# enyen/dppo

Hardware: AMD Instinct MI355X
Metric: PPO-update samples/sec (+ env-steps/sec of the K=20 sampler), hopper K=20 n_envs=512 (higher is better)
Workload: dtype bf16; 1 GPU; hopper-medium-v2 ft_ppo_diffusion_mlp K=20 Kft=10 Ta=4 (BASELINE configs[1]); n_envs_per_gpu=512, minibatch_per_gpu=50000, rollout_rows_per_gpu=256000, parallelism=dp1 (env-sharded, RCCL grad all-reduce)

## Files before the change

dppo_amd/csrc/api.hip:

```cpp
#include <math.h>
#include <stdarg.h>
#include <stdio.h>
#include <string.h>

#include "fused.h"
#include "gemm.h"
#include "ppo.h"
#include "gaussian.h"
#include "gmm.h"
#include "unet.h"
#include "sampler.h"

using namespace dppo;

static thread_local char g_err[512] = "";
static int fail(int code, const char* fmt, ...) {
  va_list ap;
  va_start(ap, fmt);
  vsnprintf(g_err, sizeof(g_err), fmt, ap);
  va_end(ap);
  return code;
}
namespace dppo {
void set_vis_mfma_attn(int v);
// ... 577 lines not shown
  return g_lowrank_top && d.n_blocks >= 1 && M >= (int64_t)g_lowrank_ratio * d.out_dim;
}
static int g_mom_rider = 0;
constexpr int64_t MOM_RIDER_MAX_N = 16384;
static int g_temb_onehot = 1;
template <class P>
static int temb_onehot_col(const dppo_net_desc& d, const PackLayout& L, int Kft, const MlpBufs<P>& B) {
  if (!g_temb_onehot || d.kind != 0 || !fused_ok<P>(d) || Kft < 1) return -1;
  if (d.cond_out > 0 && d.cond_out % 16) return -1;
  if (L.Kp0 - d.in_dim < Kft || (size_t)(d.hidden + d.time_dim) * Kft > B.part_floats) return -1;
  return d.in_dim;
}
static int g_dw0 = 1;
static int g_side_tail = 1;
static int g_tail_post = 1;
static int dw0_cols(const dppo_net_desc& d) { return d.kind == 0 ? d.act_flat + d.cond_dim : d.in_dim; }
static int dw0_nhot(const dppo_net_desc& d, int Kft) {
  const int room = 32 - dw0_cols(d);
  return d.kind != 0 ? 0 : (room >= Kft ? Kft : room);
}
template <class P>
static bool dw0_ok(const dppo_net_desc& d, int64_t M, const PackLayout& L, int Kft, const MlpBufs<P>& B, bool wants_dobs) {
  if (!g_dw0 || P::ESIZE != 2 || wants_dobs || d.cond_hidden > 0 || !g_tn_group || !g_post_one) return false;
  if (!fused_ok<P>(d) || B.tiles <= 0 || !bwd_one<P>(d, M) || !fused_dw0_shape(d) || L.Kp0 < 64) return false;
  if (d.kind == 0) {
    if (temb_onehot_col<P>(d, L, Kft, B) < 0 || !B.post_zeroed || d.in_dim != d.act_flat + d.time_dim + d.cond_dim) return false;
    if (d.act_flat % 4 || d.time_dim % 4 || 32 + d.time_dim > 64) return false;
    if (dw0_nhot(d, Kft) < Kft - 1) return false;
  } else if (d.in_dim > 32) {
    return false;
  }
  return (size_t)fused_bwd_one_grid<P>(d, M) * d.hidden * 32 <= B.slab_floats / 2;
}
template <class P>
static void flush_slabs(MlpBufs<P>& B, hipStream_t s, const SlotOuts* slots = nullptr, int slot_width = 0,
                        const LossArgs* fin = nullptr, bool defer_reduce = false) {
  if (B.tn_group.n > 0) {
    GemmTNGroup& gr = B.tn_group;
    gemm_tn_group_order(gr);
    launch_gemm_tn_group<P>(gr, s);
    gr.n = 0;
  }
  for (int i = 0; i + 1 < B.n_join; ++i) join_side(B.join_s[B.n_join - 1], B.join_s[i], B.join_idx[i]);
  if (B.n_join > 0) join_side(s, B.join_s[B.n_join - 1], B.join_idx[B.n_join - 1]);
  B.n_join = 0;
  if (defer_reduce) return;
  if (slots != nullptr || fin != nullptr) {
    TailReduce t;
    memset(&t, 0, sizeof(t));
    t.jobs = B.slab_jobs;
    if (slots != nullptr) t.colsum = B.tile_colsum, t.tiles = B.tiles, t.width = slot_width, t.slots = *slots;
    if (g_dbg & 4) t.jobs.n = 0;
    if (g_dbg & 8) t.slots.n_slots = 0;
    if (g_dbg & 16) fin = nullptr;
    launch_tail_reduce(t, fin, s);
  } else {
    launch_slab_reduce_batch(B.slab_jobs, s);
  }
  B.slab_jobs.n = 0, B.slab_used = 0;
}
template <class P>
static void weight_grad(const void* A, int lda, int N1, const void* Bm, int ldb, int N2, int64_t M, MlpBufs<P>& B,
                        float* gw, int ldgw, hipStream_t s, bool defer = false, int n2a = -1, float* gw2 = nullptr,
                        int ldgw2 = 0) {
  const bool swap = N1 <= 64 && N2 > 64;
  if (swap) {
// ... 81 lines not shown
  g.X = B.d_enc, g.W = pk + L.Wc2T, g.out_pre = B.d_cz, g.dsrc_kind = 2, g.dsrc_ld = L.C1p, g.dact = d.act;
  g.dsrc = d.act == DPPO_ACT_RELU ? B.ca : B.cz;
  launch_gemm_nt<P>(g, s);
  weight_grad<P>(B.d_cz, L.C1p, d.cond_hidden, cin, L.Kpc, d.cond_dim, M, B, grad + pl.c1w, d.cond_dim, s);
  launch_colsum<P>(B.d_cz, (int)M, d.cond_hidden, L.C1p, B.part, REDUCE_BLOCKS, grad + pl.c1b, 1.f, s);
}

template <class P>
static void mlp_backward(const dppo_net_desc& d, const float* prm, const char* pk, const PackLayout& L, int64_t M,
                         MlpBufs<P>& B, float* grad, const int32_t* krow, const dppo_step* ksteps, int Kft,
                         hipStream_t s, bool bout_done = false, int aux_idx = 1, const LossArgs* fin = nullptr) {
  const ParamLayout pl = param_layout(d);
  const int H = d.hidden, nb = d.n_blocks;
  if (fused_ok<P>(d) && B.tiles > 0) {
    FusedBwdArgs f;
    memset(&f, 0, sizeof(f));
    const FusedGeom fg = fused_geom<P>(d);
    f.bstream = (const u32x4*)(pk + L.bstream), f.d_out = B.d_out, f.ld_dout = L.Kpo, f.M = (int)M, f.KpB0 = fg.KpB0;
    f.nb = nb, f.act = d.act, f.colsum = B.tile_colsum, f.out_valid = d.out_dim;
    f.dout_slot = bout_done ? -1 : 2 * nb + 1 + (d.use_layernorm ? 4 * nb : 0);
    const bool post = false;
    f.params = prm, f.use_ln = d.use_layernorm, f.ln_stats = B.ln_stats;
    if (d.use_layernorm) fill_ln_off(d, pl, f.ln_off);
    for (int b = 0; b < nb; ++b) {
      f.m1[b] = post ? B.a2[b] : B.z1[b];
      f.m0[b] = post ? B.a1[b] : B.hpre[b];
      f.dz1[b] = B.dz1_all[b];
    }
    for (int b = 0; b <= nb; ++b) f.dh[b] = B.dh_all[b];
    const bool lowrank = lowrank_top(d, M);
    if (lowrank) f.dh[nb] = nullptr;
    const bool one = bwd_one<P>(d, M);
    f.one_block = one ? 1 : 0;
    if (g_dbg & 1)
      for (int b = 0; b <= nb; ++b) f.dh[b] = nullptr, f.dz1[b < nb ? b : 0] = nullptr;
    if (g_dbg & 32) f.dh[0] = nullptr;
    if (g_dbg & 2)
      for (int b = 0; b < nb; ++b) f.m1[b] = f.m0[b] = nullptr;
    const bool dw0 = B.dw0 && one && !(g_dbg & 33);
    const int dw0_nh = dw0 ? dw0_nhot(d, Kft) : 0;
    float* dw0_slab = nullptr;
    int dw0_grid = 0;
    if (B.dw0 && !dw0) {
      g_fused_fault = -7;
      return;
    }
    if (dw0) {
      dw0_grid = fused_bwd_one_grid<P>(d, M);
      if ((size_t)dw0_grid * H * 32 > B.slab_floats - B.slab_used) flush_slabs(B, s);
      dw0_slab = B.slab + B.slab_used;
      B.slab_used += (size_t)dw0_grid * H * 32;
      f.dh[0] = nullptr, f.dw0_slab = dw0_slab, f.xc = B.in, f.ld_xc = L.Kp0;
      f.xc_af = d.kind == 0 ? d.act_flat : 64, f.xc_skip = d.kind == 0 ? d.time_dim : 0;
      f.dw0_round = d.kind == 0 && dw0_nh < Kft ? 1 : 0;
    }
    g_fused_fault = launch_fused_backward<P>(d, f, s);
    if (g_fused_fault != 0) return;
    {
      SlotOuts so;
      memset(&so, 0, sizeof(so));
      so.n_slots = 2 * nb + 1;
      for (int b = nb - 1; b >= 0; --b) {
        so.out[nb - (b + 1)] = grad + pl.l2b[b];
        so.out[(nb + 1) + (nb - 1 - b)] = grad + pl.l1b[b];
      }
      so.out[nb] = grad + pl.b0;
      if (d.use_layernorm) {
        for (int b = nb - 1; b >= 0; --b) {
          const int ls = (2 * nb + 1) + 4 * (nb - 1 - b);
          so.out[ls] = grad + pl.n1w[b], so.out[ls + 1] = grad + pl.n1b[b];
          so.out[ls + 2] = grad + pl.n2w[b], so.out[ls + 3] = grad + pl.n2b[b];
        }
        so.n_slots += 4 * nb;
      }
      for (int i = 0; i < so.n_slots; ++i) so.n[i] = H;
      if (one) so.n[0] = 0;
      const float* s_rest = dw0 && f.dw0_round ? grad + pl.b0 : nullptr;
      if (!bout_done) so.out[so.n_slots] = grad + pl.bout, so.n[so.n_slots] = d.out_dim, ++so.n_slots;
      const int oh = d.kind == 0 ? temb_onehot_col<P>(d, L, Kft, B) : -1;
      const bool need_aux = d.kind == 0 && oh < 0;
      hipStream_t aux = aux_idx >= 0 && need_aux ? fork_side(s, aux_idx) : s;
      if (need_aux) time_embedding_grad<P>(d, prm, pk, L, M, B, B.dh_all[0], grad, krow, ksteps, Kft, aux);
      const bool merged = B.merged;
      const bool side_tail = dw0 && d.kind == 0 && oh >= 0 && aux_idx >= 0 && !need_aux && g_side_tail && g_early_join && g_post_one &&
                             B.post_zeroed && !(g_dbg & 28);
      TailReduce side_t;
      memset(&side_t, 0, sizeof(side_t));
      if (merged)
        weight_grad<P>(B.d_out, L.Kpo, d.out_dim, B.in, L.Kp0, d.in_dim, M, B, B.lowrank_u, L.Kp0, s, true);
      else
        weight_grad<P>(B.d_out, L.Kpo, d.out_dim, B.hE, H, H, M, B, grad + pl.Wout, H, s, true);
      for (int b = nb - 1; b >= 0; --b) {
        if ((lowrank || merged) && b == nb - 1)
          weight_grad<P>(B.d_out, L.Kpo, d.out_dim, B.a2[b], H, H, M, B, B.lowrank, H, s, true);
        if (!(lowrank && b == nb - 1))
          weight_grad<P>(B.dh_all[b + 1], H, H, B.a2[b], H, H, M, B, grad + pl.l2w[b], H, s, true);
        weight_grad<P>(B.dz1_all[b], H, H, B.a1[b], H, H, M, B, grad + pl.l1w[b], H, s, true);
      }
      if (dw0) {
        auto job = [&](int c0, int cols, float* out, int ldo) {
          SlabJob& j = side_tail ? side_t.jobs.j[side_t.jobs.n++] : B.slab_jobs.j[B.slab_jobs.n++];
          j.slab = dw0_slab, j.out = out, j.splits = dw0_grid, j.rows = H, j.cols = cols, j.lds = 32, j.ldo = ldo, j.transpose = 0;
          j.c0 = c0, j.wide = dw0_grid >= 32 ? 1 : 0;
        };
        if (d.kind == 0) {
          job(0, d.act_flat, grad + pl.W0, d.in_dim);
          job(d.act_flat, d.cond_dim, grad + pl.W0 + d.act_flat + d.time_dim, d.in_dim);
          job(d.act_flat + d.cond_dim, dw0_nh, B.part, Kft);
        } else {
          job(0, d.in_dim, grad + pl.W0, d.in_dim);
        }
      } else if (g_dbg & 32) {
      } else if (oh >= 0)
        weight_grad<P>(B.dh_all[0], H, H, B.in, L.Kp0, d.in_dim + Kft, M, B, grad + pl.W0, d.in_dim, s, true, d.in_dim, B.part,
                       Kft);
      else
        weight_grad<P>(B.dh_all[0], H, H, B.in, L.Kp0, d.in_dim, M, B, grad + pl.W0, d.in_dim, s, true);
      if (side_tail) {
        hipStream_t st = fork_side(s, aux_idx);
        side_t.colsum = B.tile_colsum, side_t.tiles = B.tiles, side_t.width = H, side_t.slots = so;
        launch_tail_reduce(side_t, fin, st);
        PostReduce qs;
        memset(&qs, 0, sizeof(qs));
        qs.H = H, qs.out_dim = d.out_dim;
        qs.S = B.part, qs.W0 = prm + pl.W0, qs.ldw0 = d.in_dim, qs.AF = d.act_flat, qs.Kft = Kft, qs.td = d.time_dim;
        qs.G = B.part + (size_t)H * Kft, qs.w1 = prm + pl.te1_w, qs.b1 = prm + pl.te1_b, qs.w2 = prm + pl.te2_w;
        qs.ksteps = ksteps, qs.gw1 = grad + pl.te1_w, qs.gb1 = grad + pl.te1_b, qs.gw2 = grad + pl.te2_w, qs.gb2 = grad + pl.te2_b;
        qs.S_rest = s_rest, qs.dW0t = grad + pl.W0, qs.temb = (const float*)(pk + L.temb), qs.temb_bf16 = P::ESIZE == 2 ? 1 : 0;
        qs.counter = (unsigned*)B.post_counter;
        launch_post_reduce(qs, st);
// ... 1601 lines not shown
      g_tn_max_splits = value;
      return 0;
    case 5: set_gemm_tn_variant(value); return 0;
    case 6: set_gemm_tn_thin(value); return 0;
    case 7: set_fused_short_tiles(value); return 0;
    case 8: g_dbg = value; return 0;
    case 9: case 10: return retired_knob(knob);
    case 11: g_temb_onehot = value; return 0;
    case 12: g_tn_group = value; return 0;
    case 13: g_pack_one = value; return 0;
    case 14: g_early_join = value; return 0;
    case 15: set_sampler_l0_lds(value); return 0;
    case 16: g_lowrank_top = value; return 0;
    case 17: g_merge_top = value; return 0;
    case 18: g_post_one = value; return 0;
    case 20: dppo::set_vis_mfma_attn(value); return 0;
    case 21: set_gemm_nt_small(value); return 0;
    case 22: set_fused_merge_fwd(value); return 0;
    case 23: set_fused_bwd_one(value); return 0;
    case 25: set_fused_compact(value); return 0;
    case 26: set_gemm_tn_nbuf(value); return 0;
    case 27: set_sampler_split(value); return 0;
    case 28: set_sampler_split_pre_sweep(value); return 0;
    case 29: set_sampler_split_spin_limit(value); return 0;
    case 30:
      if (value < 1) break;
      g_lowrank_ratio = value;
      return 0;
    case 31: case 32: case 33: case 34: case 35: return retired_knob(knob);
    case 36: g_mom_rider = value; return 0;
    case 37: g_dw0 = value; return 0;
    case 38: g_side_tail = value; return 0;
    case 39: case 40: return retired_knob(knob);
    case 41: g_tail_post = value; return 0;
    default: break;
  }
  return fail(-1, "unknown tuning knob %d", knob);
}

int dppo_gemm_nt_raw(int prec, const void* X, const void* W, const float* bias, int64_t M, int N, int Kp, float* out_f32,
                     void* out_elem, int ldo, int act, dppo_stream_t stream) {
  if (int e = check_prec(prec)) return e;
  if (!X || !W || M < 1 || M > 0x7fffffff || N < 1) return fail(-1, "bad argument");
  const int es = prec == DPPO_PREC_F32 ? 4 : 2;
  if (Kp < 1 || (Kp * es) % 128) return fail(-1, "Kp must be a multiple of %d", 128 / es);
  if (ldo < ((N + 15) & ~15)) return fail(-1, "ldo too small");
  GemmNT g;
  memset(&g, 0, sizeof(g));
  g.X = X, g.W = W, g.bias = bias, g.M = (int)M, g.N = N, g.Kp = Kp, g.ldx = Kp, g.ldw = Kp;
  g.out_f32 = out_f32, g.ldo32 = ldo, g.out_act = out_elem, g.ldo = ldo, g.act = act;
  if (prec == DPPO_PREC_F32)
    launch_gemm_nt<F32>(g, (hipStream_t)stream);
  else
    launch_gemm_nt<BF16>(g, (hipStream_t)stream);
  return check_launch();
}

int dppo_gemm_tn_raw(int prec, const void* A, int lda, int N1, const void* B, int ldb, int N2, int64_t M,
                     int rows_per_split, float* slab, float* C, dppo_stream_t stream) {
  if (int e = check_prec(prec)) return e;
  if (!A || !B || !slab || !C || M < 1 || M > 0x7fffffff || N1 < 1 || N2 < 1) return fail(-1, "bad argument");
  if (rows_per_split < 64 || rows_per_split % 64) return fail(-1, "rows_per_split must be a multiple of 64");
  const int es = prec == DPPO_PREC_F32 ? 4 : 2;
  if (lda < N1 || ldb < N2) return fail(-1, "lda / ldb smaller than N1 / N2");
  if ((lda * es) % 16 || (ldb * es) % 16) return fail(-1, "lda and ldb must be multiples of %d", 16 / es);
  GemmTN t;
// ... 97 lines not shown
```

dppo_amd/csrc/common.h:

```cpp
#pragma once
#include <hip/hip_runtime.h>
#include <stdint.h>

#include <atomic>

namespace dppo {

struct DevLatch {
  std::atomic<uint64_t> bits{0};
  static int dev() {
    int d = 0;
    (void)hipGetDevice(&d);
    return d & 63;
  }
  bool need() const { return !((bits.load(std::memory_order_acquire) >> dev()) & 1); }
  void done() { bits.fetch_or(1ull << dev(), std::memory_order_release); }
};

typedef __attribute__((ext_vector_type(4))) float f32x4;
typedef __attribute__((ext_vector_type(8))) __bf16 bf16x8;
typedef __attribute__((ext_vector_type(4))) short i16x4;
typedef __attribute__((ext_vector_type(4))) uint32_t u32x4;
typedef __attribute__((ext_vector_type(2))) uint32_t u32x2;

// ... 120 lines not shown
    c0 = hi1 ^ c1 ^ k0, c1 = lo1, c2 = hi0 ^ c3 ^ k1, c3 = lo0;
    k0 += 0x9E3779B9u, k1 += 0xBB67AE85u;
  }
  const float u1 = ((float)c0 + 1.f) * 2.3283064365386963e-10f;
  const float u2 = (float)c1 * 2.3283064365386963e-10f;
  return sqrtf(-2.f * __logf(u1)) * __cosf(6.283185307179586f * u2);
}

template <class T>
__device__ __forceinline__ T lds_load(const T* p) {
  return *(const __attribute__((address_space(3))) T*)p;
}
template <class T>
__device__ __forceinline__ T glb_load(const T* p) {
  return *(const __attribute__((address_space(1))) T*)p;
}

static inline int round_up(int x, int m) { return (x + m - 1) / m * m; }

__device__ __forceinline__ float row16_sum(float x) {
  x += __builtin_bit_cast(float, __builtin_amdgcn_update_dpp(0, __builtin_bit_cast(int, x), 0xB1, 0xF, 0xF, true));
  x += __builtin_bit_cast(float, __builtin_amdgcn_update_dpp(0, __builtin_bit_cast(int, x), 0x4E, 0xF, 0xF, true));
  x += __builtin_bit_cast(float, __builtin_amdgcn_update_dpp(0, __builtin_bit_cast(int, x), 0x141, 0xF, 0xF, true));
  x += __builtin_bit_cast(float, __builtin_amdgcn_update_dpp(0, __builtin_bit_cast(int, x), 0x140, 0xF, 0xF, true));
  return x;
}

template <class P>
__host__ __device__ __forceinline__ constexpr int feat_off(int g, int tp) {
  constexpr int EPC = 16 / P::ESIZE, TPC = EPC / 4;
  return (tp / TPC) * (4 * EPC) + EPC * g + 4 * (tp % TPC);
}

}
```

dppo_amd/csrc/fused.hip:

```cpp
#include <type_traits>

#include "fused.h"
#include "gemm.h"
#include "tile_ln.h"
#include "pack_dev.h"

#ifndef DPPO_BWD_LATE
#define DPPO_BWD_LATE 1
#endif
#ifndef DPPO_BWD_PREFETCH
#define DPPO_BWD_PREFETCH 1
#endif
#ifndef DPPO_FLAGS
#define DPPO_FLAGS 1
#endif

namespace dppo {

#ifdef DPPO_STAMPS
__device__ unsigned long long g_stamps[8][32];
#define STAMP(i)                                                                   \
  do {                                                                             \
    if (blockIdx.x == 0 && lane == 0 && tile == (int)gridDim.x) g_stamps[wid][i] = clock64(); \
  } while (0)
// ... 293 lines not shown
            if constexpr (round_back) {
              v[tp + (2 * e) / 4][m][(2 * e) % 4] = __uint_as_float(o[e] << 16);
              v[tp + (2 * e + 1) / 4][m][(2 * e + 1) % 4] = __uint_as_float(o[e] & 0xffff0000u);
            }
          }
          *(u32x4*)(stage + row * 64 + ((g ^ (row & 3)) << 4)) = o;
        }
        const int sr0 = 8 * g + q, sr1 = sr0 + 4;
#pragma unroll
        for (int t = 0; t < 2; ++t) {
          const int c = 2 * t + (p >> 1);
          const u32x2 u0 = lds_tr16(stage + sr0 * 64 + ((c ^ (sr0 & 3)) << 4) + (p & 1) * 8);
          const u32x2 u1 = lds_tr16(stage + sr1 * 64 + ((c ^ (sr1 & 3)) << 4) + (p & 1) * 8);
          fa[ks][t] = (u32x4){u0.x, u0.y, u1.x, u1.y};
        }
        asm volatile("" ::: "memory");
      }
#pragma unroll
      for (int t = 0; t < 2; ++t) {
#pragma unroll
        for (int nt = 0; nt < 2; ++nt) {
          f32x4* cp = cacc + ((tp + t) * 2 + nt) * 64 + lane;
          f32x4 c = *cp;
          c = BF16::mma(fa[0][t], xb[0][nt], c);
          c = BF16::mma(fa[1][t], xb[1][nt], c);
          *cp = c;
        }
        asm volatile("" ::: "memory");
      }
    }
  }
}

constexpr int SIGN_WORDS = 32;

template <class P, int TPW, int MR>
__device__ __forceinline__ void emit(const f32x4 (&v)[TPW][MR], int actk, char* lds, void* glb, int H, int wbase, int g,
                                     int r, int row0, int M, void* dglb = nullptr) {
  constexpr int ES = P::ESIZE;
  const int HRB = H * ES;
  asm volatile("" : "+v"(r), "+v"(g));
  with_act(actk, [&](auto tag) {
    constexpr int ACT = decltype(tag)::value;
    auto body = [&](auto grad_tag) {
    constexpr bool with_grad = decltype(grad_tag)::value;
    constexpr bool with_mask = with_grad && ACT == ACT_RELU;
#pragma unroll
    for (int m = 0; m < MR; ++m) {
      const int grow = row0 + 16 * m + r;
      const bool live = grow < M;
      char* gp = glb != nullptr && live ? (char*)glb + (size_t)grow * HRB : nullptr;
      char* dp = with_grad && !with_mask && live ? (char*)dglb + (size_t)grow * HRB : nullptr;
      uint32_t bits = 0;
      char* lp = lds != nullptr ? lds + (16 * m + r) * HRB : nullptr;
      constexpr int TPC = ES == 4 ? 1 : 2;
#pragma unroll
      for (int tp = 0; tp < TPW; tp += TPC) {
        float av[4 * TPC], dv[4 * TPC];
        if constexpr (ACT == ACT_MISH) {
#pragma unroll
          for (int q = 0; q < 4 * TPC; q += 2) {
            const float2v x = {v[tp + q / 4][m][q % 4], v[tp + (q + 1) / 4][m][(q + 1) % 4]};
            float2v a2, d2;
            mish_both2(x, a2, d2);
            av[q] = a2.x, av[q + 1] = a2.y;
            dv[q] = with_grad ? d2.x : 0.f, dv[q + 1] = with_grad ? d2.y : 0.f;
          }
// ... 1185 lines not shown
```

dppo_amd/csrc/gemm.h:

```cpp
#pragma once
#include "common.h"

namespace dppo {

struct GemmNT {
  const void* X;
  const void* W;
  const float* bias;
  int M, N, Kp;
  int ldx, ldw;
  const void* dsrc;
  int dsrc_kind, dsrc_ld, dact;
  const float* res;
  int ldres;
  const void* add;
  int ldadd;
  float* out_f32;
  int ldo32;
  void* out_pre;
  void* out_act;
  int ldo, act;
};

struct GemmTN {
  const void* A;
  const void* B;
  int M, N1, N2, lda, ldb;
  float* slab;
  int ldc, splits, rows_per_split;
  int ncol_a, ncol_b;
};

constexpr int MAX_TN_JOBS = 8;
struct GemmTNGroup {
  GemmTN j[MAX_TN_JOBS];
  int base[MAX_TN_JOBS + 1];
  int n;
};

template <class P>
void launch_gemm_nt(const GemmNT& a, hipStream_t s);
template <class P>
void launch_gemm_tn_group(const GemmTNGroup& gr, hipStream_t s);
void gemm_tn_group_order(GemmTNGroup& gr);
void set_gemm_tn_variant(int v);
void set_gemm_tn_nbuf(int v);
void set_gemm_tn_thin(int v);

enum { PROBE_GEMM_NT_HIDDEN = 1, PROBE_GEMM_TN = 2, PROBE_FUSED_FWD = 3, PROBE_FUSED_BWD = 4, PROBE_SAMPLER = 5 };
void set_gemm_nt_variant(int v);
void set_gemm_nt_small(int v);
int probe_arm(int kernel_id, int max_launches);
int probe_collect(double* total_ms, int* launches, double* flops, double* bytes = nullptr);
bool probe_begin(int kernel_id, hipStream_t s);
void probe_end(hipStream_t s, double flops, double bytes = 0);
template <class P>
void launch_gemm_tn(const GemmTN& a, hipStream_t s);
bool gemm_tn_thin(int N1, int N2);

void launch_slab_reduce(const float* slab, int splits, size_t n, float* out, float scale, hipStream_t s);
template <class P>
void launch_colsum(const void* A, int M, int N, int lda, float* partial , int blocks, float* out,
                   float scale, hipStream_t s);
// ... 3 lines not shown
```

dppo_amd/csrc/gemm.hip:

```cpp
#include "gemm.h"

namespace dppo {

template <class P, int WN, int WM, int TN, int TM, int TAG, int DMA>
__global__ __launch_bounds__(WN* WM * 64) void gemm_nt_kernel(const GemmNT a) {
  typedef typename P::elem_t E;
  constexpr int BN = WN * TN * 16, BM = WM * TM * 16, T = WN * WM * 64, ES = P::ESIZE;
  constexpr int NW = (BN * 8 + T - 1) / T, NX = (BM * 8 + T - 1) / T;
  constexpr int STAGE = (BN + BM) * 128;
  extern __shared__ __attribute__((aligned(16))) char smem[];

  const int tid = threadIdx.x, lane = tid & 63, wid = tid >> 6;
  const int r = lane & 15, g = lane >> 4;
  const int wn = wid % WN, wm = wid / WN;
  const int row0 = blockIdx.x * BM, feat0 = blockIdx.y * BN;
  const char* Xb = (const char*)a.X;
  const char* Wb = (const char*)a.W;
  const int nk = a.Kp * ES / 128;

  u32x4 wreg[NW], xreg[NX];
  auto gload = [&](int kt) {
#pragma unroll
    for (int i = 0; i < NW; ++i) {
      const int q = (tid + i * T) % (BN * 8);
// ... 239 lines not shown
template <class P>
void launch_gemm_nt(const GemmNT& a, hipStream_t s) {
  if (a.M <= 0) return;
  const bool dma = g_nt_variant == 1 && a.N % 128 == 0;
  const int64_t wg128 = (int64_t)((a.M + 127) / 128) * ((a.N + 127) / 128);
  if (g_nt_small && a.N > 16 && wg128 < 192) {
    const bool dma64 = g_nt_variant == 1 && a.N % 64 == 0;
    const int64_t wg64 = (int64_t)((a.M + 63) / 64) * ((a.N + 63) / 64);
    if (wg64 >= 192) {
      if (dma64) launch_nt_cfg<P, 2, 2, 2, 2, 0, 1>(a, s);
      else launch_nt_cfg<P, 2, 2, 2, 2, 0, 0>(a, s);
    } else {
      if (dma64) launch_nt_cfg<P, 2, 2, 2, 1, 0, 1>(a, s);
      else launch_nt_cfg<P, 2, 2, 2, 1, 0, 0>(a, s);
    }
    return;
  }
  if (a.N <= 16)
    launch_nt_cfg<P, 1, 4, 1, 4, 0, 0>(a, s);
  else if (a.N <= 64)
    launch_nt_cfg<P, 1, 4, 4, 2, 0, 0>(a, s);
  else if (a.N == a.Kp && dma)
    launch_nt_cfg<P, 2, 2, 4, 4, 1, 1>(a, s);
  else if (a.N == a.Kp)
    launch_nt_cfg<P, 2, 2, 4, 4, 1, 0>(a, s);
  else if (dma)
    launch_nt_cfg<P, 2, 2, 4, 4, 0, 1>(a, s);
  else
    launch_nt_cfg<P, 2, 2, 4, 4, 0, 0>(a, s);
}
template void launch_gemm_nt<F32>(const GemmNT&, hipStream_t);
template void launch_gemm_nt<BF16>(const GemmNT&, hipStream_t);

template <class P, int WA, int WB, int TA, int TB, int NBUF = 2>
__device__ __forceinline__ void tn_tile(const GemmTN& a, const int split, const int fa0, const int fb0) {
  constexpr int ES = P::ESIZE;
  constexpr int BA = WA * TA * 16, BB = WB * TB * 16;
  constexpr int ROWS = (ES == 2) ? 64 : 32;
  constexpr int RSA = BA * ES + 32, RSB = BB * ES + 32;
  constexpr int CPA = BA * ES / 16, CPB = BB * ES / 16;
  constexpr int NCA = (ROWS * CPA + 255) / 256, NCB = (ROWS * CPB + 255) / 256;
  constexpr int OPA = ROWS * RSA, OPB = ROWS * RSB;
  extern __shared__ __attribute__((aligned(16))) char smem[];

  const int tid = threadIdx.x, lane = tid & 63, wid = tid >> 6;
  const int r = lane & 15, g = lane >> 4;
  const int wa = wid % WA, wb = wid / WA;
  const int m_begin = split * a.rows_per_split;
  const int m_end = min(a.M, m_begin + a.rows_per_split);
  const char* Ab = (const char*)a.A;
  const char* Bb = (const char*)a.B;

  u32x4 areg[NCA], breg[NCB];
  const int lim_a = a.ncol_a > 0 ? a.ncol_a : a.lda, lim_b = a.ncol_b > 0 ? a.ncol_b : a.ldb;
  auto gload = [&](int m0) {
#pragma unroll
    for (int i = 0; i < NCA; ++i) {
      const int q = (tid + i * 256) % (ROWS * CPA);
      const int rr = q / CPA, c = q % CPA;
      const int row = m0 + rr, ca = fa0 + c * (16 / ES);
      areg[i] = (u32x4){0, 0, 0, 0};
      if (row < m_end && ca < lim_a) areg[i] = *(const u32x4*)(Ab + ((size_t)row * a.lda + ca) * ES);
    }
#pragma unroll
    for (int i = 0; i < NCB; ++i) {
      const int q = (tid + i * 256) % (ROWS * CPB);
      const int rr = q / CPB, c = q % CPB;
      const int row = m0 + rr, cb = fb0 + c * (16 / ES);
      breg[i] = (u32x4){0, 0, 0, 0};
      if (row < m_end && cb < lim_b) breg[i] = *(const u32x4*)(Bb + ((size_t)row * a.ldb + cb) * ES);
    }
  };
  auto sstore = [&](int st) {
    char* As = smem + st * (OPA + OPB);
    char* Bs = As + OPA;
#pragma unroll
    for (int i = 0; i < NCA; ++i) {
      const int q = (tid + i * 256) % (ROWS * CPA);
      *(u32x4*)(As + (q / CPA) * RSA + (q % CPA) * 16) = areg[i];
    }
#pragma unroll
    for (int i = 0; i < NCB; ++i) {
      const int q = (tid + i * 256) % (ROWS * CPB);
      *(u32x4*)(Bs + (q / CPB) * RSB + (q % CPB) * 16) = breg[i];
    }
  };

  f32x4 acc[TA][TB];
#pragma unroll
  for (int i = 0; i < TA; ++i)
#pragma unroll
    for (int j = 0; j < TB; ++j) acc[i][j] = (f32x4){0.f, 0.f, 0.f, 0.f};

  const int nst = (m_end - m_begin + ROWS - 1) / ROWS;
  if (nst > 0) {
    gload(m_begin);
    sstore(0);
  }
  __syncthreads();
  for (int st = 0; st < nst; ++st) {
    const int cur = NBUF == 2 ? (st & 1) : 0;
    if (st + 1 < nst) gload(m_begin + (st + 1) * ROWS);
    const char* As = smem + cur * (OPA + OPB);
    const char* Bs = As + OPA;
#pragma unroll
    for (int s = 0; s < 2; ++s) {
      u32x4 af[TA], bf[TB];
      if constexpr (ES == 2) {
        typedef __attribute__((address_space(3))) i16x4 lds_v;
        const int q = r >> 2, p = r & 3;
        const int rbase = 32 * s + 8 * g;
        const int r0 = rbase + ((g & 1) ? 4 : 0) + q, r1 = rbase + ((g & 1) ? 0 : 4) + q;
#pragma unroll
        for (int t = 0; t < TA; ++t) {
          const int ca = (wa * TA * 16 + t * 16 + 4 * p) * 2;
          const u32x2 u0 = __builtin_bit_cast(u32x2, __builtin_amdgcn_ds_read_tr16_b64_v4i16((lds_v*)(As + r0 * RSA + ca)));
          const u32x2 u1 = __builtin_bit_cast(u32x2, __builtin_amdgcn_ds_read_tr16_b64_v4i16((lds_v*)(As + r1 * RSA + ca)));
          af[t] = (u32x4){u0.x, u0.y, u1.x, u1.y};
        }
#pragma unroll
        for (int t = 0; t < TB; ++t) {
          const int cb = (wb * TB * 16 + t * 16 + 4 * p) * 2;
          const u32x2 u0 = __builtin_bit_cast(u32x2, __builtin_amdgcn_ds_read_tr16_b64_v4i16((lds_v*)(Bs + r0 * RSB + cb)));
          const u32x2 u1 = __builtin_bit_cast(u32x2, __builtin_amdgcn_ds_read_tr16_b64_v4i16((lds_v*)(Bs + r1 * RSB + cb)));
          bf[t] = (u32x4){u0.x, u0.y, u1.x, u1.y};
        }
      } else {
#pragma unroll
        for (int t = 0; t < TA; ++t) {
          const int ca = (wa * TA * 16 + t * 16 + r) * 4;
          uint32_t v[4];
#pragma unroll
          for (int j = 0; j < 4; ++j) v[j] = *(const uint32_t*)(As + (16 * s + 4 * j + g) * RSA + ca);
          af[t] = (u32x4){v[0], v[1], v[2], v[3]};
        }
#pragma unroll
        for (int t = 0; t < TB; ++t) {
          const int cb = (wb * TB * 16 + t * 16 + r) * 4;
          uint32_t v[4];
#pragma unroll
          for (int j = 0; j < 4; ++j) v[j] = *(const uint32_t*)(Bs + (16 * s + 4 * j + g) * RSB + cb);
          bf[t] = (u32x4){v[0], v[1], v[2], v[3]};
        }
      }
#pragma unroll
      for (int i = 0; i < TA; ++i)
#pragma unroll
        for (int j = 0; j < TB; ++j) acc[i][j] = P::mma(af[i], bf[j], acc[i][j]);
    }
    if constexpr (NBUF == 1) __syncthreads();
    if (st + 1 < nst) sstore(NBUF == 2 ? cur ^ 1 : 0);
    __syncthreads();
  }

  float* out = a.slab + (size_t)split * a.N1 * a.ldc;
#pragma unroll
  for (int i = 0; i < TA; ++i)
#pragma unroll
    for (int e = 0; e < 4; ++e) {
      const int n1 = fa0 + wa * TA * 16 + i * 16 + 4 * g + e;
      if (n1 >= a.N1) continue;
#pragma unroll
      for (int j = 0; j < TB; ++j) {
        const int n2 = fb0 + wb * TB * 16 + j * 16 + r;
        if (n2 < a.N2) out[(size_t)n1 * a.ldc + n2] = acc[i][j][e];
      }
    }
}

template <class P, int WA, int WB, int TA, int TB>
__global__ __launch_bounds__(256) void gemm_tn_kernel(const GemmTN a) {
  tn_tile<P, WA, WB, TA, TB>(a, blockIdx.x, blockIdx.y * (WA * TA * 16), blockIdx.z * (WB * TB * 16));
}

template <class P, int NBUF>
__global__ __launch_bounds__(256, NBUF == 1 ? 3 : 2) void gemm_tn_group_kernel(const GemmTNGroup gr) {
  const int bid = blockIdx.x;
  int j = 0;
#pragma unroll
  for (int i = 1; i < MAX_TN_JOBS; ++i)
    if (i < gr.n && bid >= gr.base[i]) j = i;
  const GemmTN& a = gr.j[j];
  const int local = bid - gr.base[j];
  const int split = local % a.splits, tile = local / a.splits;
  const int tb = (a.N2 + 127) / 128;
  const int fa0 = (tile / tb) * 128, fb0 = (tile % tb) * 128;
  tn_tile<P, 2, 2, 4, 4, NBUF>(a, split, fa0, fb0);
}

__device__ u32x4 g_zero_chunk[1];
template <int CP>
__device__ __forceinline__ constexpr int swz(int q) {
  return CP >= 16 ? (q & 7) << 1 : (CP >= 8 ? (q & 3) << 1 : 0);
}

template <class P, int WA, int WB, int TA, int TB, int NST, int KS>
__global__ __launch_bounds__(WA* WB * 64) void gemm_tn_dma_kernel(const GemmTN a) {
  constexpr int ES = P::ESIZE, NT = WA * WB * 64;
  constexpr int BA = WA * TA * 16, BB = WB * TB * 16;
  constexpr int ROWS = KS * ((ES == 2) ? 32 : 16);
  constexpr int RSA = BA * ES, RSB = BB * ES;
  constexpr int CPA = RSA / 16, CPB = RSB / 16;
  static_assert(CPA >= 8 && CPB >= 8 && (ROWS * CPA) % NT == 0 && (ROWS * CPB) % NT == 0, "tile / thread-count mismatch");
  constexpr int NCA = ROWS * CPA / NT, NCB = ROWS * CPB / NT, NLD = NCA + NCB;
  constexpr int OPA = ROWS * RSA, STAGE = ROWS * (RSA + RSB);
  extern __shared__ __attribute__((aligned(16))) char smem[];
  typedef __attribute__((address_space(3))) void* lds_ptr;
  typedef const __attribute__((address_space(1))) void* glb_ptr;

  const int tid = threadIdx.x, lane = tid & 63, wid = tid >> 6;
  const int r = lane & 15, g = lane >> 4;
  const int wa = wid % WA, wb = wid / WA;
  const int fa0 = blockIdx.y * BA, fb0 = blockIdx.z * BB;
  const int m_begin = blockIdx.x * a.rows_per_split;
  const int m_end = min(a.M, m_begin + a.rows_per_split);
  const char* Ab = (const char*)a.A;
  const char* Bb = (const char*)a.B;
  const char* zero = (const char*)g_zero_chunk;

  auto dma = [&](int stage_idx, int buf) {
// ... 111 lines not shown
  if (attr_set.need()) {
    (void)hipFuncSetAttribute((const void*)gemm_tn_dma_kernel<P, WA, WB, TA, TB, NST, KS>,
                              hipFuncAttributeMaxDynamicSharedMemorySize, LDS);
    attr_set.done();
  }
  const bool probe = a.N1 >= 128 && a.N2 >= 128 && probe_begin(PROBE_GEMM_TN, s);
  hipLaunchKernelGGL((gemm_tn_dma_kernel<P, WA, WB, TA, TB, NST, KS>), grid, dim3(WA * WB * 64), LDS, s, a);
  if (probe) probe_end(s, 2.0 * a.M * a.N1 * a.N2);
}

template <class P, int WA, int WB, int TA, int TB>
static void launch_tn_cfg(const GemmTN& a, hipStream_t s) {
  constexpr int ES = P::ESIZE, BA = WA * TA * 16, BB = WB * TB * 16, ROWS = (ES == 2) ? 64 : 32;
  constexpr int LDS = 2 * ROWS * ((BA * ES + 32) + (BB * ES + 32));
  dim3 grid(a.splits, (a.N1 + BA - 1) / BA, (a.N2 + BB - 1) / BB);
  static DevLatch attr_set;
  if (attr_set.need()) {
    (void)hipFuncSetAttribute((const void*)gemm_tn_kernel<P, WA, WB, TA, TB>, hipFuncAttributeMaxDynamicSharedMemorySize,
                              LDS);
    attr_set.done();
  }
  const bool probe = BA == 128 && a.N1 >= 128 && a.N2 >= 128 && probe_begin(PROBE_GEMM_TN, s);
  hipLaunchKernelGGL((gemm_tn_kernel<P, WA, WB, TA, TB>), grid, dim3(256), LDS, s, a);
  if (probe) probe_end(s, 2.0 * a.M * a.N1 * a.N2);
}

static int g_tn_nbuf = 0;
void set_gemm_tn_nbuf(int v) { g_tn_nbuf = v == 2 ? 2 : (v == 1 ? 1 : 0); }
template <class P>
void launch_gemm_tn_group(const GemmTNGroup& gr, hipStream_t s) {
  if (gr.n <= 0) return;
  constexpr int ES = P::ESIZE, ROWS = (ES == 2) ? 64 : 32;
  constexpr int LDS = 2 * ROWS * 2 * (128 * ES + 32);
  static DevLatch attr_set;
  if (attr_set.need()) {
    (void)hipFuncSetAttribute((const void*)gemm_tn_group_kernel<P, 2>, hipFuncAttributeMaxDynamicSharedMemorySize, LDS);
    attr_set.done();
  }
  double flops = 0, bytes = 0;
  for (int i = 0; i < gr.n; ++i) {
    const GemmTN& a = gr.j[i];
    flops += 2.0 * a.M * a.N1 * a.N2;
    bytes += (double)a.M * (a.N1 + a.N2) * ES + 4.0 * a.N1 * a.N2;
  }
  const bool probe = probe_begin(PROBE_GEMM_TN, s);
  const dim3 grid(gr.base[gr.n]);
  const int nbuf = g_tn_nbuf != 0 ? g_tn_nbuf : ((int)grid.x > 3 * 256 && gr.n > 0 && gr.j[0].M >= 32768 ? 2 : 1);
  if (nbuf == 1)
    hipLaunchKernelGGL((gemm_tn_group_kernel<P, 1>), grid, dim3(256), LDS / 2, s, gr);
  else
    hipLaunchKernelGGL((gemm_tn_group_kernel<P, 2>), grid, dim3(256), LDS, s, gr);
  if (probe) probe_end(s, flops, bytes);
}
void gemm_tn_group_order(GemmTNGroup& gr) {
  for (int i = 1; i < gr.n; ++i)
    for (int k = i; k > 0 && gr.j[k].rows_per_split > gr.j[k - 1].rows_per_split; --k) {
      const GemmTN t = gr.j[k];
      gr.j[k] = gr.j[k - 1], gr.j[k - 1] = t;
    }
  gr.base[0] = 0;
  for (int i = 0; i < gr.n; ++i) {
    const int tiles = ((gr.j[i].N1 + 127) / 128) * ((gr.j[i].N2 + 127) / 128);
    gr.base[i + 1] = gr.base[i] + gr.j[i].splits * tiles;
  }
}
template void launch_gemm_tn_group<F32>(const GemmTNGroup&, hipStream_t);
template void launch_gemm_tn_group<BF16>(const GemmTNGroup&, hipStream_t);

static int g_tn_thin = 1;
void set_gemm_tn_thin(int v) { g_tn_thin = v; }
bool gemm_tn_thin(int N1, int N2) { return g_tn_thin && N2 <= 64 && N1 > 64; }

static int g_tn_variant = 0;
void set_gemm_tn_variant(int v) { g_tn_variant = v; }

template <class P>
void launch_gemm_tn(const GemmTN& a, hipStream_t s) {
  if (a.ncol_a > 0 || a.ncol_b > 0) {
    launch_tn_cfg<P, 2, 2, 4, 4>(a, s);
    return;
// ... 96 lines not shown
```

Baseline: 143.5 million samples/s.

## Rebuild first-layer dz1 inside the weight-grad GEMM instead of storing it

```diff
diff --git a/dppo_amd/csrc/api.hip b/dppo_amd/csrc/api.hip
--- a/dppo_amd/csrc/api.hip
+++ b/dppo_amd/csrc/api.hip
@@ -633,6 +633,12 @@
   }
   return (size_t)fused_bwd_one_grid<P>(d, M) * d.hidden * 32 <= B.slab_floats / 2;
 }
+static int g_dw1_rebuild = 1;
+template <class P>
+static bool dw1_rebuild(const dppo_net_desc& d, int64_t M, const MlpBufs<P>& B) {
+  return g_dw1_rebuild && P::ESIZE == 2 && g_tn_group && !g_dbg && fused_ok<P>(d) && B.tiles > 0 && bwd_one<P>(d, M) &&
+         d.act == DPPO_ACT_RELU && !d.use_layernorm && d.out_dim <= 32 && d.hidden == 512;
+}
 template <class P>
 static void flush_slabs(MlpBufs<P>& B, hipStream_t s, const SlotOuts* slots = nullptr, int slot_width = 0,
                         const LossArgs* fin = nullptr, bool defer_reduce = false) {
@@ -780,6 +786,8 @@
     if (lowrank) f.dh[nb] = nullptr;
     const bool one = bwd_one<P>(d, M);
     f.one_block = one ? 1 : 0;
+    const bool rebuild = dw1_rebuild<P>(d, M, B);
+    if (rebuild) f.dz1[0] = nullptr;
     if (g_dbg & 1)
       for (int b = 0; b <= nb; ++b) f.dh[b] = nullptr, f.dz1[b < nb ? b : 0] = nullptr;
     if (g_dbg & 32) f.dh[0] = nullptr;
@@ -843,7 +851,12 @@
           weight_grad<P>(B.d_out, L.Kpo, d.out_dim, B.a2[b], H, H, M, B, B.lowrank, H, s, true);
         if (!(lowrank && b == nb - 1))
           weight_grad<P>(B.dh_all[b + 1], H, H, B.a2[b], H, H, M, B, grad + pl.l2w[b], H, s, true);
-        weight_grad<P>(B.dz1_all[b], H, H, B.a1[b], H, H, M, B, grad + pl.l1w[b], H, s, true);
+        weight_grad<P>(rebuild ? nullptr : B.dz1_all[b], H, H, B.a1[b], H, H, M, B, grad + pl.l1w[b], H, s, true);
+        if (rebuild) {
+          GemmTN& t = B.tn_group.j[B.tn_group.n - 1];
+          t.pa_w = f.bstream, t.pa_dout = B.d_out, t.pa_ld = L.Kpo, t.pa_sign = (const uint32_t*)B.z1[b];
+          t.pa_pos = fg.KSB0, t.pa_total = fg.total_pos;
+        }
       }
       if (dw0) {
         auto job = [&](int c0, int cols, float* out, int ldo) {
@@ -2511,6 +2524,7 @@
     case 37: g_dw0 = value; return 0;
     case 38: g_side_tail = value; return 0;
     case 39: case 40: return retired_knob(knob);
+    case 42: g_dw1_rebuild = value; return 0;
     case 41: g_tail_post = value; return 0;
     default: break;
   }
diff --git a/dppo_amd/csrc/common.h b/dppo_amd/csrc/common.h
--- a/dppo_amd/csrc/common.h
+++ b/dppo_amd/csrc/common.h
@@ -176,4 +176,8 @@
   return (tp / TPC) * (4 * EPC) + EPC * g + 4 * (tp % TPC);
 }
 
+constexpr int SIGN_WORDS = 32;
+__host__ __device__ __forceinline__ constexpr int sign_word_bf16(int f, int tpw) { return f / (16 * tpw) * 4 + (f % 32) / 8; }
+__host__ __device__ __forceinline__ constexpr int sign_bit_bf16(int f, int tpw) { return (f % (16 * tpw)) / 32 * 8 + f % 8; }
+
 }
diff --git a/dppo_amd/csrc/fused.hip b/dppo_amd/csrc/fused.hip
--- a/dppo_amd/csrc/fused.hip
+++ b/dppo_amd/csrc/fused.hip
@@ -349,7 +349,6 @@
   }
 }
 
-constexpr int SIGN_WORDS = 32;
 
 template <class P, int TPW, int MR>
 __device__ __forceinline__ void emit(const f32x4 (&v)[TPW][MR], int actk, char* lds, void* glb, int H, int wbase, int g,
diff --git a/dppo_amd/csrc/gemm.h b/dppo_amd/csrc/gemm.h
--- a/dppo_amd/csrc/gemm.h
+++ b/dppo_amd/csrc/gemm.h
@@ -29,6 +29,10 @@
   float* slab;
   int ldc, splits, rows_per_split;
   int ncol_a, ncol_b;
+  const u32x4* pa_w;
+  const void* pa_dout;
+  const uint32_t* pa_sign;
+  int pa_ld, pa_pos, pa_total;
 };
 
 constexpr int MAX_TN_JOBS = 8;
diff --git a/dppo_amd/csrc/gemm.hip b/dppo_amd/csrc/gemm.hip
--- a/dppo_amd/csrc/gemm.hip
+++ b/dppo_amd/csrc/gemm.hip
@@ -295,7 +295,7 @@
 template void launch_gemm_nt<F32>(const GemmNT&, hipStream_t);
 template void launch_gemm_nt<BF16>(const GemmNT&, hipStream_t);
 
-template <class P, int WA, int WB, int TA, int TB, int NBUF = 2>
+template <class P, int WA, int WB, int TA, int TB, int NBUF = 2, int PROD = 0>
 __device__ __forceinline__ void tn_tile(const GemmTN& a, const int split, const int fa0, const int fb0) {
   constexpr int ES = P::ESIZE;
   constexpr int BA = WA * TA * 16, BB = WB * TB * 16;
@@ -316,14 +316,46 @@
 
   u32x4 areg[NCA], breg[NCB];
   const int lim_a = a.ncol_a > 0 ? a.ncol_a : a.lda, lim_b = a.ncol_b > 0 ? a.ncol_b : a.ldb;
+  constexpr bool CAN_PROD = PROD != 0 && ES == 2 && BA == 128 && NCA == 4;
+  static_assert(PROD == 0 || CAN_PROD || ES != 2, "operand producers: bf16, 128-feature A tiles");
+  static_assert(sign_word_bf16(64 + 32 + 8, 4) == 4 + 1 && sign_bit_bf16(64 + 32 + 8 + 5, 4) == 8 + 5, "sign-word layout (common.h)");
+  const bool pa = CAN_PROD && a.pa_w != nullptr;
+  u32x4 paw[CAN_PROD ? 2 : 1];
+  uint32_t psg[2] = {0, 0};
+  char* const SD = smem + NBUF * (OPA + OPB);
+  char* const SS = SD + ROWS * 64;
+  char* const SW = SS + ROWS * 32;
+  if constexpr (CAN_PROD) {
+    if (pa) {
+      const int fw = fa0 + 32 * wid;
+      const u32x4* w = a.pa_w + ((size_t)(fw / 64) * a.pa_total + a.pa_pos) * 4 * 64 + (fw % 64) / 32 * 2 * 64 + lane;
+      paw[0] = w[0], paw[1] = w[64];
+      if constexpr (NBUF == 1) {
+        *(u32x4*)(SW + (2 * wid) * 1024 + lane * 16) = paw[0];
+        *(u32x4*)(SW + (2 * wid + 1) * 1024 + lane * 16) = paw[1];
+      }
+    }
+  }
   auto gload = [&](int m0) {
-#pragma unroll
-    for (int i = 0; i < NCA; ++i) {
-      const int q = (tid + i * 256) % (ROWS * CPA);
-      const int rr = q / CPA, c = q % CPA;
-      const int row = m0 + rr, ca = fa0 + c * (16 / ES);
-      areg[i] = (u32x4){0, 0, 0, 0};
-      if (row < m_end && ca < lim_a) areg[i] = *(const u32x4*)(Ab + ((size_t)row * a.lda + ca) * ES);
+    if (pa) {
+      if constexpr (CAN_PROD) {
+        const int row = m0 + (tid >> 2), c = tid & 3;
+        areg[0] = (u32x4){0, 0, 0, 0}, psg[0] = psg[1] = 0;
+        if (row < m_end) {
+          areg[0] = *(const u32x4*)((const char*)a.pa_dout + ((size_t)row * a.pa_ld + 8 * c) * 2);
+          const u32x2 sw = *(const u32x2*)(a.pa_sign + (size_t)row * SIGN_WORDS + (fa0 / 64) * 8 + 2 * c);
+          psg[0] = sw.x, psg[1] = sw.y;
+        }
+      }
+    } else {
+#pragma unroll
+      for (int i = 0; i < NCA; ++i) {
+        const int q = (tid + i * 256) % (ROWS * CPA);
+        const int rr = q / CPA, c = q % CPA;
+        const int row = m0 + rr, ca = fa0 + c * (16 / ES);
+        areg[i] = (u32x4){0, 0, 0, 0};
+        if (row < m_end && ca < lim_a) areg[i] = *(const u32x4*)(Ab + ((size_t)row * a.lda + ca) * ES);
+      }
     }
 #pragma unroll
     for (int i = 0; i < NCB; ++i) {
@@ -334,13 +366,51 @@
       if (row < m_end && cb < lim_b) breg[i] = *(const u32x4*)(Bb + ((size_t)row * a.ldb + cb) * ES);
     }
   };
+  auto stage_put = [&]() {
+    if constexpr (CAN_PROD) {
+      if (pa) {
+        int t_ = tid;
+        asm volatile("" : "+v"(t_));
+        const int row = t_ >> 2, c = t_ & 3;
+        *(u32x4*)(SD + row * 64 + ((c ^ ((row >> 2) & 3)) << 4)) = areg[0];
+        *(u32x2*)(SS + row * 32 + c * 8) = (u32x2){psg[0], psg[1]};
+      }
+    }
+  };
   auto sstore = [&](int st) {
     char* As = smem + st * (OPA + OPB);
     char* Bs = As + OPA;
-#pragma unroll
-    for (int i = 0; i < NCA; ++i) {
-      const int q = (tid + i * 256) % (ROWS * CPA);
-      *(u32x4*)(As + (q / CPA) * RSA + (q % CPA) * 16) = areg[i];
+    if (pa) {
+      if constexpr (CAN_PROD) {
+        int r = lane & 15, g = lane >> 4, lane_ = lane;
+        asm volatile("" : "+v"(r), "+v"(g), "+v"(lane_));
+#pragma unroll
+        for (int m = 0; m < 4; ++m) {
+          const int rr = 16 * m + r;
+          const u32x4 xb = *(const u32x4*)(SD + rr * 64 + ((g ^ ((rr >> 2) & 3)) << 4));
+          const f32x4 z = (f32x4){0.f, 0.f, 0.f, 0.f};
+          const u32x4 w0 = NBUF == 1 ? *(const u32x4*)(SW + (2 * wid) * 1024 + lane_ * 16) : paw[0];
+          const u32x4 w1 = NBUF == 1 ? *(const u32x4*)(SW + (2 * wid + 1) * 1024 + lane_ * 16) : paw[1];
+          f32x4 c[2] = {P::mma(w0, xb, z), P::mma(w1, xb, z)};
+          const uint32_t bits = *(const uint32_t*)(SS + rr * 32 + ((wid >> 1) * 4 + g) * 4) >> (8 * (wid & 1));
+          u32x4 o;
+#pragma unroll
+          for (int t = 0; t < 2; ++t) {
+#pragma unroll
+            for (int e = 0; e < 4; ++e) c[t][e] *= (bits >> (4 * t + e)) & 1u ? 1.f : 0.f;
+            o[2 * t] = (uint32_t)f2bf(c[t][0]) | ((uint32_t)f2bf(c[t][1]) << 16);
+            o[2 * t + 1] = (uint32_t)f2bf(c[t][2]) | ((uint32_t)f2bf(c[t][3]) << 16);
+          }
+          *(u32x4*)(As + (16 * m + r) * RSA + (32 * wid + 8 * g) * 2) = o;
+          __builtin_amdgcn_sched_barrier(0);
+        }
+      }
+    } else {
+#pragma unroll
+      for (int i = 0; i < NCA; ++i) {
+        const int q = (tid + i * 256) % (ROWS * CPA);
+        *(u32x4*)(As + (q / CPA) * RSA + (q % CPA) * 16) = areg[i];
+      }
     }
 #pragma unroll
     for (int i = 0; i < NCB; ++i) {
@@ -358,6 +428,8 @@
   const int nst = (m_end - m_begin + ROWS - 1) / ROWS;
   if (nst > 0) {
     gload(m_begin);
+    stage_put();
+    if (pa) __syncthreads();
     sstore(0);
   }
   __syncthreads();
@@ -411,7 +483,11 @@
 #pragma unroll
         for (int j = 0; j < TB; ++j) acc[i][j] = P::mma(af[i], bf[j], acc[i][j]);
     }
-    if constexpr (NBUF == 1) __syncthreads();
+    if (st + 1 < nst) stage_put();
+    if constexpr (NBUF == 1)
+      __syncthreads();
+    else if (pa)
+      __syncthreads();
     if (st + 1 < nst) sstore(NBUF == 2 ? cur ^ 1 : 0);
     __syncthreads();
   }
@@ -436,7 +512,7 @@
   tn_tile<P, WA, WB, TA, TB>(a, blockIdx.x, blockIdx.y * (WA * TA * 16), blockIdx.z * (WB * TB * 16));
 }
 
-template <class P, int NBUF>
+template <class P, int NBUF, int PROD = 0>
 __global__ __launch_bounds__(256, NBUF == 1 ? 3 : 2) void gemm_tn_group_kernel(const GemmTNGroup gr) {
   const int bid = blockIdx.x;
   int j = 0;
@@ -448,7 +524,7 @@
   const int split = local % a.splits, tile = local / a.splits;
   const int tb = (a.N2 + 127) / 128;
   const int fa0 = (tile / tb) * 128, fb0 = (tile % tb) * 128;
-  tn_tile<P, 2, 2, 4, 4, NBUF>(a, split, fa0, fb0);
+  tn_tile<P, 2, 2, 4, 4, NBUF, PROD>(a, split, fa0, fb0);
 }
 
 __device__ u32x4 g_zero_chunk[1];
@@ -626,20 +702,40 @@
   if (gr.n <= 0) return;
   constexpr int ES = P::ESIZE, ROWS = (ES == 2) ? 64 : 32;
   constexpr int LDS = 2 * ROWS * 2 * (128 * ES + 32);
+  constexpr int PROD_LDS = ROWS * (64 + 32);
   static DevLatch attr_set;
   if (attr_set.need()) {
     (void)hipFuncSetAttribute((const void*)gemm_tn_group_kernel<P, 2>, hipFuncAttributeMaxDynamicSharedMemorySize, LDS);
     attr_set.done();
   }
   double flops = 0, bytes = 0;
+  bool prod = false;
   for (int i = 0; i < gr.n; ++i) {
     const GemmTN& a = gr.j[i];
     flops += 2.0 * a.M * a.N1 * a.N2;
-    bytes += (double)a.M * (a.N1 + a.N2) * ES + 4.0 * a.N1 * a.N2;
-  }
-  const bool probe = probe_begin(PROBE_GEMM_TN, s);
+    const double a_row = a.pa_w != nullptr ? 64.0 + 4.0 * SIGN_WORDS : (double)a.N1 * ES;
+    bytes += (double)a.M * (a_row + (double)a.N2 * ES) + 4.0 * a.N1 * a.N2;
+    prod = prod || a.pa_w != nullptr;
+  }
   const dim3 grid(gr.base[gr.n]);
   const int nbuf = g_tn_nbuf != 0 ? g_tn_nbuf : ((int)grid.x > 3 * 256 && gr.n > 0 && gr.j[0].M >= 32768 ? 2 : 1);
+  if (prod) {
+    if constexpr (ES == 2) {
+      static DevLatch attr_prod;
+      if (attr_prod.need()) {
+        (void)hipFuncSetAttribute((const void*)gemm_tn_group_kernel<P, 2, 1>, hipFuncAttributeMaxDynamicSharedMemorySize, LDS + PROD_LDS);
+        attr_prod.done();
+      }
+      const bool probe = probe_begin(PROBE_GEMM_TN, s);
+      if (nbuf == 1)
+        hipLaunchKernelGGL((gemm_tn_group_kernel<P, 1, 1>), grid, dim3(256), LDS / 2 + PROD_LDS + 8192, s, gr);
+      else
+        hipLaunchKernelGGL((gemm_tn_group_kernel<P, 2, 1>), grid, dim3(256), LDS + PROD_LDS, s, gr);
+      if (probe) probe_end(s, flops, bytes);
+    }
+    return;
+  }
+  const bool probe = probe_begin(PROBE_GEMM_TN, s);
   if (nbuf == 1)
     hipLaunchKernelGGL((gemm_tn_group_kernel<P, 1>), grid, dim3(256), LDS / 2, s, gr);
   else
```

Result: slower. 133.8 million samples/s (-6.7%).
